# honglianghe/CDNet

Hardware: AMD Instinct MI355X
Metric: tiles/sec (train fwd+bwd+Adam), 256x256 (higher is better)
Workload: dtype fp32

## Files before the change

cdnet_amd/csrc/bn_bwd.hip:

```cpp
#include "train_util.h"
#include "bn_sums.h"

using namespace cdnet;

namespace {

struct GradIn {
    const unsigned short *g;
    int Hg, Wg;
    int oy, ox;
    int pooled;
    int coff, cstride;
};

struct BnBwdArgs {
    const unsigned short *raw;
    const unsigned short *res;
    int f16;
    const float *scale, *shift;
    int relu;
    const float *mean, *invstd;
    GradIn gin[3];
    int ngin;
    int N, H, W, C;
    float *partial;
    const float *k1, *k2, *k3;
    unsigned short *draw;
    unsigned short *dz_out;
    int rev;
};


__device__ __forceinline__ void act8_f32(const BnBwdArgs &A, size_t e, const float *sc, const float *sh, float *a, float *rawf) {
    float x[8], r[8];
    ldf8(A.raw, e, x);
    if (A.res) ldf8(A.res, e, r);
#pragma unroll
    for (int j = 0; j < 8; ++j) {
        if (rawf) rawf[j] = x[j];
        float v = A.scale ? fmaf(x[j], sc[j], sh[j]) : x[j];
        if (A.relu == 2) v = r[j];
        else {
            if (A.res) v += r[j];
            if (A.relu) v = fmaxf(v, 0.f);
// ... 286 lines not shown
                if (APPLY) {
                    if (valid) {
                        const unsigned pw = rev ? npix - 1 - p : p;
                        *reinterpret_cast<uint4 *>(A.draw + (size_t)pw * A.C + c0) = o.u;
                        if (RES) *reinterpret_cast<uint4 *>(A.dz_out + (size_t)pw * A.C + c0) = z.u;
                    }
                } else {
                    if (RES && A.dz_out && valid) *reinterpret_cast<uint4 *>(A.dz_out + (size_t)p * A.C + c0) = res[u].u;
                }
            }
        }
    });
    if (!APPLY) bn_write_partial<8>(A.partial, A.C, VPP, s1, s2);
}

template <int NG, bool RES, bool APPLY>
__global__ __launch_bounds__(256) void bn_bwd_flat32_kernel(BnBwdArgs A) {
    const int VPP = A.C / 4;
    const int slot = (int)threadIdx.x % VPP, c0 = slot * 4;
    float sc[4], sh[4], mu[4], is[4], k1[4], k2[4], k3[4], s1[4], s2[4];
    bn_load_row<4>(A.scale, c0, sc, 1.f); bn_load_row<4>(A.shift, c0, sh, 0.f); bn_load_row<4>(A.mean, c0, mu, 0.f); bn_load_row<4>(A.invstd, c0, is, 1.f);
    if (APPLY) { bn_load_row<4>(A.k1, c0, k1, 1.f); bn_load_row<4>(A.k2, c0, k2, 0.f); bn_load_row<4>(A.k3, c0, k3, 0.f); }
#pragma unroll
    for (int j = 0; j < 4; ++j) { s1[j] = 0.f; s2[j] = 0.f; }
    const unsigned npix = (unsigned)(A.N * A.H * A.W);
    const unsigned ppb = 256 / VPP, step = gridDim.x * ppb;
    const bool relu = A.relu != 0, outmask = A.relu == 2;
    const float *raw = reinterpret_cast<const float *>(A.raw), *resp = reinterpret_cast<const float *>(A.res);
    float *draw = reinterpret_cast<float *>(A.draw), *dzo = reinterpret_cast<float *>(A.dz_out);
    for (unsigned p0 = first_pixel(ppb, VPP); p0 < npix; p0 += step * BN_U) {
        f32x4 x[BN_U], r[BN_U], g[BN_U][NG];
#pragma unroll
        for (int u = 0; u < BN_U; ++u) {
            unsigned p = p0 + u * step;
            p = p < npix ? p : npix - 1;
            if (APPLY && A.rev) p = npix - 1 - p;
            x[u] = *reinterpret_cast<const f32x4 *>(raw + (size_t)p * A.C + c0);
            if (RES) r[u] = *reinterpret_cast<const f32x4 *>(resp + (size_t)p * A.C + c0);
#pragma unroll
            for (int k = 0; k < NG; ++k)
                g[u][k] = *reinterpret_cast<const f32x4 *>(reinterpret_cast<const float *>(A.gin[k].g) + (size_t)p * A.gin[k].cstride + A.gin[k].coff + c0);
        }
#pragma unroll
        for (int u = 0; u < BN_U; ++u) {
            const unsigned p = p0 + u * step;
            const bool valid = p < npix;
            f32x4 o, z;
#pragma unroll
            for (int j = 0; j < 4; ++j) {
                float v = fmaf(x[u][j], sc[j], sh[j]);
                if (RES) v = outmask ? r[u][j] : v + r[u][j];
                float gs = g[u][0][j];
#pragma unroll
                for (int k = 1; k < NG; ++k) gs += g[u][k][j];
                const float dz = (!valid || (relu && !(v > 0.f))) ? 0.f : gs;
                const float xh = (x[u][j] - mu[j]) * is[j];
                if (APPLY) { o[j] = k1[j] * (dz - k2[j] - xh * k3[j]); z[j] = dz; }
                else { s1[j] += dz; s2[j] = fmaf(dz, xh, s2[j]); z[j] = dz; }
            }
            if (APPLY && valid) {
                const unsigned pw = A.rev ? npix - 1 - p : p;
                *reinterpret_cast<f32x4 *>(draw + (size_t)pw * A.C + c0) = o;
                if (RES) *reinterpret_cast<f32x4 *>(dzo + (size_t)pw * A.C + c0) = z;
            }
            if (!APPLY && RES && dzo && valid) *reinterpret_cast<f32x4 *>(dzo + (size_t)p * A.C + c0) = z;
        }
    }
    if (!APPLY) bn_write_partial<4>(A.partial, A.C, VPP, s1, s2);
}

// ... 155 lines not shown
static int fill_bn_args(const cdnet_bn_bwd_args *a, BnBwdArgs &A, const char *who) {
    CDNET_REQUIRE(a && a->raw, "%s: null pointer", who);
    CDNET_REQUIRE(a->C % 8 == 0 && a->C >= 8 && a->C <= 2048 , "%s: C=%d unsupported", who, a->C);
    CDNET_REQUIRE(a->ngin >= 1 && a->ngin <= 3, "%s: ngin=%d", who, a->ngin);
    A.raw = a->raw; A.res = a->res; A.f16 = a->f16; A.scale = a->scale; A.shift = a->shift; A.relu = a->relu;
    A.mean = a->mean; A.invstd = a->invstd;
    for (int k = 0; k < 3; ++k) {
        A.gin[k].g = a->gin[k].g; A.gin[k].Hg = a->gin[k].Hg; A.gin[k].Wg = a->gin[k].Wg;
        A.gin[k].oy = a->gin[k].oy; A.gin[k].ox = a->gin[k].ox; A.gin[k].pooled = a->gin[k].pooled;
        A.gin[k].coff = a->gin[k].coff; A.gin[k].cstride = a->gin[k].cstride ? a->gin[k].cstride : a->C;
        if (k < a->ngin) CDNET_REQUIRE(a->gin[k].g, "%s: null gradient input %d", who, k);
        if (k < a->ngin) CDNET_REQUIRE(a->gin[k].Hg >= 1 && a->gin[k].Wg >= 1, "%s: empty gradient input %d (%d x %d)", who, k, a->gin[k].Hg, a->gin[k].Wg);
    }
    A.ngin = a->ngin; A.N = a->N; A.H = a->H; A.W = a->W; A.C = a->C;
    A.partial = nullptr; A.k1 = A.k2 = A.k3 = nullptr; A.draw = nullptr; A.dz_out = nullptr;
    return CDNET_OK;
}

enum BnPath { BN_WINDOW, BN_FLAT, BN_GENERIC };
struct BnPlan {
    BnPath path;
    bool f32;
    int nb;
    int kp, nflat;
    bool flat_sources;
};

static size_t bn_npix(const BnBwdArgs &A) { return (size_t)A.N * A.H * A.W; }

static BnPlan bn_plan_plain(const BnBwdArgs &A) {
// ... 18 lines not shown
    if (window && (!f32 || (fits32 && A.shift && A.invstd))) P.path = BN_WINDOW;
    else if (flat && (!f32 || fits32)) P.path = BN_FLAT;
    const int V = f32 && P.path != BN_GENERIC ? 4 : 8;
    P.nb = window ? bn_grid((size_t)A.N * ((A.H + 1) / 2) * ((A.W + 1) / 2), A.C, V, 1) : bn_grid(bn_npix(A), A.C, V, BN_U);
    return P;
}

static thread_local int g_bn_last_plan[2] = {0, 0};
static thread_local int g_bn_last_pass = 0;

static int bn_plan_record(const BnPlan &P, const BnBwdArgs &A, bool apply, bool dz_source) {
    const int path = P.path == BN_WINDOW ? CDNET_BN_PATH_WINDOW : P.path == BN_FLAT ? CDNET_BN_PATH_FLAT : CDNET_BN_PATH_GENERIC;
    const int n = P.path == BN_WINDOW ? P.nflat : P.path == BN_FLAT ? A.ngin : 0;
    const int res = P.path == BN_FLAT && A.res ? 1 : 0;
    const int kp = P.path == BN_WINDOW ? P.kp : 0;
    return path | (P.f32 ? 1 : 0) << 2 | n << 3 | res << 5 | kp << 6 | (apply ? 1 : 0) << 8 | (dz_source ? 1 : 0) << 9 | P.nb << 10;
}

template <bool APPLY>
static void launch(const BnPlan &P, const BnBwdArgs &A, hipStream_t st, bool dz_source = false) {
    g_bn_last_plan[APPLY ? 1 : 0] = bn_plan_record(P, A, APPLY, dz_source);
    g_bn_last_pass = APPLY ? 1 : 0;
    auto window = [&](auto nf) {
        constexpr int NF = decltype(nf)::value;
        if (P.f32) bn_bwd_window32_kernel<NF, APPLY><<<P.nb, 256, 0, st>>>(A, P.kp);
        else bn_bwd_window_kernel<NF, APPLY><<<P.nb, 256, 0, st>>>(A, P.kp);
    };
    auto flat = [&](auto ng, auto res) {
        constexpr int NG = decltype(ng)::value;
        constexpr bool RES = decltype(res)::value;
        if (P.f32) bn_bwd_flat32_kernel<NG, RES, APPLY><<<P.nb, 256, 0, st>>>(A);
        else bn_bwd_flat_kernel<NG, RES, APPLY><<<P.nb, 256, 0, st>>>(A);
    };
    using std::integral_constant;
    using std::true_type;
    using std::false_type;
    switch (P.path) {
        case BN_WINDOW:
            if (P.nflat == 0) window(integral_constant<int, 0>{});
            else if (P.nflat == 1) window(integral_constant<int, 1>{});
            else window(integral_constant<int, 2>{});
            break;
        case BN_FLAT:
            switch (A.ngin * 2 + (A.res ? 1 : 0)) {
                case 2: flat(integral_constant<int, 1>{}, false_type{}); break;
                case 3: flat(integral_constant<int, 1>{}, true_type{}); break;
// ... 24 lines not shown
    B.gin[0].coff = 0; B.gin[0].cstride = A.C;
    B.res = nullptr; B.relu = 0; B.dz_out = nullptr;
    return B;
}

extern "C" int cdnet_bn_backward(const cdnet_bn_bwd_args *a, const float *gamma, float *dgamma, float *dbeta, float *workspace,
                                 size_t workspace_floats, uint16_t *draw, uint16_t *dz_out, void *stream) {
    BnBwdArgs A;
    int rc = fill_bn_args(a, A, "cdnet_bn_backward");
    if (rc) return rc;
    hipStream_t st = (hipStream_t)stream;
    const size_t npix = bn_npix(A);
    CDNET_REQUIRE(npix * (size_t)A.C < ((size_t)1 << 32) && npix < ((size_t)1 << 31), "cdnet_bn_backward: tensor too large for 32-bit pixel indexing");
    const BnPlan P = bn_plan(A, draw, dz_out);
    CDNET_REQUIRE(A.relu != 2 || (P.flat_sources && A.res), "cdnet_bn_backward: relu = 2 (mask from the stored output) needs same-size gradient sources and res");
    static const bool dz_reuse = !(getenv("CDNET_BN_DZ_REUSE") && atoi(getenv("CDNET_BN_DZ_REUSE")) == 0);
    const bool reuse = dz_reuse && P.path == BN_FLAT && A.mean && A.res && dz_out;
    A.draw = draw;
    A.rev = 1;
    if (A.mean) {
        CDNET_REQUIRE(gamma && A.invstd && workspace, "cdnet_bn_backward: BatchNorm layer needs gamma/invstd/workspace");
        const size_t need = (size_t)P.nb * 2 * A.C + 3 * (size_t)A.C;
        if (workspace_floats < need) { set_error("cdnet_bn_backward: workspace %zu < %zu floats", workspace_floats, need); return CDNET_E_WORKSPACE; }
        A.partial = workspace;
        A.dz_out = dz_reuse ? dz_out : nullptr;
        float *k = workspace + (size_t)P.nb * 2 * A.C;
        launch<false>(P, A, st);
        bn_finalize(A, A.partial, P.nb, gamma, dgamma, dbeta, k, st);
        bn_set_coeffs(A, k);
    }
// ... 59 lines not shown
```

cdnet_amd/csrc/conv.hip:

```cpp
#include <type_traits>
#include <vector>
#include "common.h"
#include "conv_args.h"
#include "launch.h"
#include "xform.h"
#include "stage16.h"
#include <stdlib.h>

using namespace cdnet;

namespace {

__device__ int g_dbg_dummy;

struct PackDesc {
    const float *w;
    unsigned short *out;
    int Cout, Cin, KH, KW, CK, BN, nchunk, ntile, TAPS, mode, parity;
    unsigned block0, nblocks;
    int split;
    const float *scale;
};

__device__ __forceinline__ void pack_range(const PackDesc &d, size_t first, size_t stride) {
// ... 1324 lines not shown
    CDNET_REQUIRE(A.N > 0 && A.H > 0 && A.W > 0 && A.Cout > 0 && A.Cout % 8 == 0, "cdnet_conv_forward: bad size (Cout must be a multiple of 8)");
    {
        int ctot_xf = 0;
        for (int i = 0; i < A.nsrc; ++i) ctot_xf += A.src[i].C;
        CDNET_REQUIRE(ctot_xf <= XF_MAX, "cdnet_conv_forward: %d source channels exceed the %d-entry scale/shift table", ctot_xf, XF_MAX);
    }
    CDNET_REQUIRE(A.ws == 0 || A.ws == 2, "cdnet_conv_forward: ws must be 0 or 2 (BatchNorm-backward statistics epilogue)");
    if (A.f32) {
        CDNET_REQUIRE(A.f32 == 1, "cdnet_conv_forward: f32 must be 0 or 1");
        for (int i = 0; i < A.nsrc; ++i)
            CDNET_REQUIRE(A.src[i].f16 == 2, "cdnet_conv_forward(f32): every source must be fp32 (f16 = 2)");
    } else {
        for (int i = 0; i < A.nsrc; ++i)
            CDNET_REQUIRE(A.src[i].f16 == 0 || A.src[i].f16 == 1, "cdnet_conv_forward: fp32 sources need args.f32 = 1");
    }
    if (A.eres && A.ws != 2) {
        CDNET_REQUIRE(A.ostride == 1 && A.npar == 1 && A.out_coff == 0 && A.out_cstride == A.Cout && !A.stats && !A.orelu &&
                      !A.out_f16 && ((A.eres_scale == nullptr) == (A.eres_shift == nullptr)),
                      "cdnet_conv_forward: fused residual epilogue needs a dense bf16 output, no statistics and no ReLU before the add");
    }
    int nchunk = 0;
    for (int i = 0; i < A.nsrc; ++i) {
        CDNET_REQUIRE(A.src[i].x && A.src[i].C % A.CK == 0, "cdnet_conv_forward: source %d channels %d not a multiple of CK=%d",
                      i, A.src[i].C, A.CK);
        CDNET_REQUIRE(!(A.src[i].pool && A.src[i].res), "cdnet_conv_forward: pool+residual source unsupported");
        nchunk += A.src[i].C / A.CK;
    }
    const bool padded = A.nchunk == nchunk + 1 && A.taps == 9 && A.nsrc == 2 && !A.f32;
    CDNET_REQUIRE(nchunk == A.nchunk || padded, "cdnet_conv_forward: nchunk %d != %d", A.nchunk, nchunk);
    CDNET_REQUIRE((A.taps == 9 && A.npar == 1 && A.ostride == 1) || (A.taps == 1 && A.npar == 1 && A.ostride == 1) ||
// ... 56 lines not shown
```

cdnet_amd/csrc/conv32.hip:

```cpp
#include <type_traits>
#include "common.h"
#include "conv_args.h"
#include "launch.h"
#include "split_bf16.h"
#include <stdlib.h>

using namespace cdnet;

namespace {

constexpr int CK = 16;
constexpr int PSTR = CK * 2 + 16;
constexpr int XF_MAX = 2048;

template <int TH, int TW, int BN, int TAPS>
struct Lds32 {
    static constexpr int NPIX = (TH + 2) * (TW + 2);
    static constexpr int A_PLANE = NPIX * PSTR;
    static constexpr int B_PLANE = TAPS * CK * BN * 2;
    static constexpr int STAGE = 2 * A_PLANE + 2 * B_PLANE;
    static constexpr int STATS_BYTES = 4 * 2 * BN * 4;
    static constexpr int MAIN = ((STAGE > STATS_BYTES ? STAGE : STATS_BYTES) + 15) / 16 * 16;
    static int bytes(int ctot) { return MAIN + 2 * ((ctot + 7) / 8 * 8) * 4; }
};
// ... 348 lines not shown
    const int smem = L::bytes(ctot);
    dim3 grid(cdiv(A.W, TW) * cdiv(A.H, TH) * A.N * A.npar, cdiv(A.Cout, BN), 1);
    g_conv_last_form = conv_form(CDNET_CONV_FAMILY_F32, BN, TAPS, 0, false, false, false, 0, 0, TH);
    return launch_lds<conv_f32_kernel<TH, TW, BN, WM, WN, TAPS>>(grid, 256, L::bytes(XF_MAX), smem, st, "hipFuncSetAttribute(conv32)", "conv_f32_kernel", A);
}

template <int TAPS>
int dispatch_conv32(const ConvArgs &A, hipStream_t st) {
    if (A.tile == 16 && A.BN == 64) return launch_conv32<16, 16, 64, 4, 1, TAPS>(A, st);
    if (A.tile == 16 && A.BN == 32) return launch_conv32<16, 16, 32, 4, 1, TAPS>(A, st);
    if (A.tile == 8 && A.BN == 64) return launch_conv32<8, 8, 64, 2, 2, TAPS>(A, st);
    set_error("cdnet_conv_forward(f32): unsupported configuration tile=%d CK=%d BN=%d", A.tile, A.CK, A.BN);
    return CDNET_E_ARG;
}

template <int BN, int NCH, bool XF, bool ERES>
__global__ __launch_bounds__(256, 4) void conv1x1_f32_stream_kernel(ConvArgs A) {
    constexpr int NPW = BN / 32;
    constexpr int B_PLANE = CK * BN * 2;
    constexpr int CIN = NCH * CK;
    __shared__ __attribute__((aligned(16))) unsigned char smem[NCH * 2 * B_PLANE + 2 * CIN * 4];
    unsigned char *lds_b = smem;
    float *s_xf = reinterpret_cast<float *>(smem + NCH * 2 * B_PLANE);

    const int tid = threadIdx.x, lane = tid & 63, wave = __builtin_amdgcn_readfirstlane(tid >> 6);
    const int half = lane >> 5, l31 = lane & 31;
    const int cout_tile = blockIdx.y, cout0 = cout_tile * BN;
    const ConvSrc &S = A.src[0];
    {
        const u32x4 *wsrc = reinterpret_cast<const u32x4 *>(A.w + (size_t)cout_tile * NCH * B_PLANE);
        u32x4 *bdst = reinterpret_cast<u32x4 *>(lds_b);
        for (int v = tid; v < NCH * 2 * B_PLANE / 16; v += 256) bdst[v] = wsrc[v];
// ... 83 lines not shown
        const size_t left = P - (size_t)blk * 32, rows = left < 32 ? left : 32;
        const __amdgpu_buffer_rsrc_t ro = rsrc(obase + (size_t)blk * 32 * cs4, rows * cs4);
        float ev[NPW][16];
        if (ERES) {
            const __amdgpu_buffer_rsrc_t re = rsrc(ebase + (size_t)blk * 32 * ce4, rows * ce4);
#pragma unroll
            for (int ni = 0; ni < NPW; ++ni)
#pragma unroll
                for (int r = 0; r < 16; ++r) {
                    const unsigned pr = (r & 3) + 8 * (r >> 2);
                    ev[ni][r] = __builtin_bit_cast(float, TAIL ? __builtin_amdgcn_raw_buffer_load_b32(re, (int)(vo_eres[ni] + pr * ce4), 0, 0)
                                                               : __builtin_amdgcn_raw_buffer_load_b32(re, (int)vo_eres[ni], (int)(pr * ce4), 0));
                }
        }
#pragma unroll
        for (int ni = 0; ni < NPW; ++ni)
#pragma unroll
            for (int r = 0; r < 16; ++r) {
                const unsigned pr = (r & 3) + 8 * (r >> 2);
                float v = fmaf(acc[ni][r], osc[ni], osh[ni]);
                v = orelu ? fmaxf(v, 0.f) : v;
                if (ERES) {
                    v = fmaf(ev[ni][r], esc[ni], esh[ni]) + v;
                    v = eres_relu ? fmaxf(v, 0.f) : v;
                }
                if (TAIL) __builtin_amdgcn_raw_buffer_store_b32(__builtin_bit_cast(unsigned, v), ro, (int)(vo_out[ni] + pr * cs4), 0, 0);
                else __builtin_amdgcn_raw_buffer_store_b32(__builtin_bit_cast(unsigned, v), ro, (int)vo_out[ni], (int)(pr * cs4), 0);
            }
    };
    f32x4 xa[NCH][2], xb[NCH][2];
    const int nfull = (int)(P / 32);
    if (blk < nfull) {
        request(xa, blk);
#pragma unroll
        for (int c = 0; c < NCH; ++c) asm volatile("" ::"v"(xa[c][0]), "v"(xa[c][1]));
        for (;;) {
            block(std::false_type{}, xa, xb);
            blk += bstride;
            if (blk >= nfull) break;
            block(std::false_type{}, xb, xa);
            blk += bstride;
            if (blk >= nfull) break;
        }
// ... 3 lines not shown
        block(std::true_type{}, xa, xb);
    }
}

template <int BN, int NCH>
int launch_conv1x1_stream(const ConvArgs &A, hipStream_t st) {
    int n_cu = 0;
    if (const int rc = cu_count(&n_cu)) return rc;
    const long long nblk = ((long long)A.N * A.H * A.W + 31) / 32;
    const int ctiles = cdiv(A.Cout, BN);
    const long long waves = (long long)n_cu * 16 / ctiles > 4 ? (long long)n_cu * 16 / ctiles : 4;
    const long long rounds = (nblk + waves - 1) / waves;
    const long long G = ((nblk + rounds - 1) / rounds + 3) / 4;
    dim3 grid((unsigned)G, ctiles, 1);
    return with_bool(A.src[0].scale != nullptr, [&](auto xf_c) {
        return with_bool(A.eres != nullptr, [&](auto er_c) {
            g_conv_last_form = conv_form(CDNET_CONV_FAMILY_STREAM, BN, 1, decltype(xf_c)::value ? 1 : 0, false, false, false, 0, 0, 16, 16, NCH, decltype(er_c)::value);
            conv1x1_f32_stream_kernel<BN, NCH, decltype(xf_c)::value, decltype(er_c)::value><<<grid, 256, 0, st>>>(A);
            return check_launch("conv1x1_f32_stream_kernel");
        });
    });
}

int try_conv1x1_stream(const ConvArgs &A, hipStream_t st) {
    if (A.debug & CONV_DBG_NO_STREAM_1X1) return -1;
    if (A.taps != 1 || A.taps1 != 0 || A.npar != 1 || A.ostride != 1 || A.ws || A.stats || A.pool_out || A.nsrc != 1) return -1;
    const ConvSrc &s = A.src[0];
    if (s.off_y || s.off_x || s.Hs != A.H || s.Ws != A.W || (s.row_stride && s.row_stride != s.Ws * s.C) || s.pool || s.res) return -1;
    if (s.relu && !s.scale) return -1;
    if (s.C != A.nchunk * CK || (long long)A.N * A.H * A.W > (1LL << 31) - 64 || (long long)A.out_cstride * 4 * 36 >= (1LL << 31)) return -1;
    auto go = [&](auto bn_c) -> int {
        constexpr int BN = decltype(bn_c)::value;
        if (A.nchunk == 1) return launch_conv1x1_stream<BN, 1>(A, st);
        if (A.nchunk == 2) return launch_conv1x1_stream<BN, 2>(A, st);
        if (A.nchunk == 4) return launch_conv1x1_stream<BN, 4>(A, st);
        return -1;
    };
    if (A.BN == 64) return go(std::integral_constant<int, 64>{});
    if (A.BN == 32) return go(std::integral_constant<int, 32>{});
    return -1;
}

__global__ __launch_bounds__(256) void materialize_f32_kernel(const ConvSrc s, int N, int H, int W, float *__restrict__ out) {
    const int VPP = s.C / 4;
    const size_t total = (size_t)N * H * W * VPP;
// ... 42 lines not shown
            }
        }
        *reinterpret_cast<float4 *>(out + pix * s.C + c) = val;
    }
}

}

namespace cdnet {

int conv_forward_f32(const ConvArgs &A, hipStream_t st) {
    CDNET_REQUIRE(A.CK == 16, "cdnet_conv_forward(f32): CK must be 16 (got %d)", A.CK);
    for (int i = 0; i < A.nsrc; ++i)
        CDNET_REQUIRE(!A.src[i].pool, "cdnet_conv_forward(f32): pooled sources must be materialised (cdnet_src_materialize)");
    CDNET_REQUIRE(!A.out_f16, "cdnet_conv_forward(f32): out_f16 must be 0");
    {
        const int rc = conv_forward_f32_ws(A, st);
        if (rc >= 0) return rc;
    }
    CDNET_REQUIRE(A.ws != 2, "cdnet_conv_forward(f32): the BatchNorm-backward statistics epilogue (ws = 2) needs the producer / consumer kernel "
                             "(ask cdnet_conv_ws_eligible first)");
    CDNET_REQUIRE(A.taps1 == 0 || A.taps1 == A.taps, "cdnet_conv_forward(f32): a one-tap second source runs on conv_ws32_kernel only (ask cdnet_conv_ws_eligible)");
    CDNET_REQUIRE(!A.pool_out, "cdnet_conv_forward(f32): the fused max-pool output rides in conv_ws32_kernel's epilogue only (ask cdnet_conv_ws_eligible)");
    if (A.taps == 9) return dispatch_conv32<9>(A, st);
    if (A.taps == 4) return dispatch_conv32<4>(A, st);
    {
        const int rc = try_conv1x1_stream(A, st);
        if (rc >= 0) return rc;
    }
    return dispatch_conv32<1>(A, st);
// ... 12 lines not shown
```

cdnet_amd/csrc/conv_args.h:

```cpp
#pragma once
#include "../../include/cdnet_hip.h"

struct ConvSrc {
    const unsigned short *x;
    const unsigned short *res;
    const float *scale;
    const float *shift;
    int C, Hs, Ws, pool, relu, off_y, off_x;
    int f16, row_stride;
};

struct ConvArgs {
    ConvSrc src[2];
    int nsrc;
    const unsigned short *w;
    const float *bias;
    const float *oscale;
    const float *oshift;
    int orelu;
    unsigned short *out;
    int Cout, out_cstride, out_coff;
    float *stats;
    int N, H, W;
    int taps, npar, ostride, nchunk;
    int tile, CK, BN;
    int out_f16;
    int debug;
    int ws;
    int f32;
    const unsigned short *eres;
    const float *eres_scale, *eres_shift;
    int eres_f16, eres_relu;
    int taps1, pad_;
    unsigned short *pool_out;
    const float *dot_w, *dot_b;
    float *dot_out;
};

enum : int {
    CONV_DBG_WS16_QUAD = 16,
    CONV_DBG_ONE_TILE = 32,
    CONV_DBG_PERSIST_SMALL = 64,
    CONV_DBG_OLD_WS16 = 128,
    CONV_DBG_NO_STREAM_1X1 = 256,
    CONV_DBG_GRID_SHIFT = 8,
};
enum : int {
    WGRAD_DBG_NO_WS = 8,
    WGRAD_DBG_ALL_QUADS = 16,
};

// ... 17 lines not shown
```

cdnet_amd/engine.py:

```python
import ctypes as C
import os
import torch

from . import _lib


class ConvSrc(C.Structure):
    _fields_ = [('x', C.c_void_p), ('res', C.c_void_p), ('scale', C.c_void_p), ('shift', C.c_void_p),
                ('C', C.c_int), ('Hs', C.c_int), ('Ws', C.c_int), ('pool', C.c_int), ('relu', C.c_int),
                ('off_y', C.c_int), ('off_x', C.c_int), ('f16', C.c_int), ('row_stride', C.c_int)]


class ConvArgs(C.Structure):
    _fields_ = [('src', ConvSrc * 2), ('nsrc', C.c_int), ('w', C.c_void_p), ('bias', C.c_void_p),
                ('oscale', C.c_void_p), ('oshift', C.c_void_p), ('orelu', C.c_int), ('out', C.c_void_p),
                ('Cout', C.c_int), ('out_cstride', C.c_int), ('out_coff', C.c_int), ('stats', C.c_void_p),
                ('N', C.c_int), ('H', C.c_int), ('W', C.c_int), ('taps', C.c_int), ('npar', C.c_int),
                ('ostride', C.c_int), ('nchunk', C.c_int), ('tile', C.c_int), ('CK', C.c_int), ('BN', C.c_int),
                ('out_f16', C.c_int), ('debug', C.c_int), ('ws', C.c_int), ('f32', C.c_int),
                ('eres', C.c_void_p), ('eres_scale', C.c_void_p), ('eres_shift', C.c_void_p), ('eres_f16', C.c_int), ('eres_relu', C.c_int),
                ('taps1', C.c_int), ('pad_', C.c_int), ('pool_out', C.c_void_p),
                ('dot_w', C.c_void_p), ('dot_b', C.c_void_p), ('dot_out', C.c_void_p)]


def _dp(t):
    return None if t is None else t.data_ptr()


class Src:

    def __init__(self, x, scale=None, shift=None, relu=False, pool=False, res=None, off=(0, 0), view=None):
        assert x.dtype in (torch.bfloat16, torch.float16, torch.float32) and x.is_contiguous()
        assert res is None or res.dtype == x.dtype
        self.x, self.scale, self.shift, self.relu, self.pool, self.res, self.off = x, scale, shift, relu, pool, res, off
        if view is None:
            assert x.dim() == 4
            self.N, self.Hs, self.Ws, self.Cc = x.shape
# ... 140 lines not shown
    if cout_scale is not None:
        assert mode == 0 and cout_scale.dtype == torch.float32 and cout_scale.numel() == Cout
        _lib.call('cdnet_pack_conv_weights_scaled', _lib.ptr(w), _lib.ptr(cout_scale), _lib.ptr(out), Cout, Cin, KH, KW, CK, BN,
                  mode | (PACK_SPLIT if split else 0), _lib.stream_ptr())
        return out
    _lib.call('cdnet_pack_conv_weights', _lib.ptr(w), _lib.ptr(out), Cout, Cin, KH, KW, CK, BN, mode | (PACK_SPLIT if split else 0),
              _lib.stream_ptr())
    return out


CONV_DEBUG = 0


def conv_forward(srcs, wpacked, Cout, cfg, taps=9, transposed=False, bias=None, oscale=None, oshift=None,
                 orelu=False, out=None, stats=None, H=None, W=None, out_dtype=torch.bfloat16, eres=None, query_ws=False, bns=None, taps1=0, pool_out=None, dot=None,
                 pad_chunks=0, debug_or=0, out_coff=0):
    tile, CK, BN = cfg[:3]
    s0 = srcs[0]
    f32 = s0.f32
    assert all(s.f32 == f32 for s in srcs)
    if f32:
        out_dtype = torch.float32
    N = s0.N
    if H is None:
        H, W = s0.logical_hw()
        H, W = H + 0, W + 0
    ostride = 2 if transposed else 1
    npar = 4 if transposed else 1
    a = ConvArgs()
    nchunk = 0
    for i, s in enumerate(srcs):
# ... 25 lines not shown
    a.debug = CONV_DEBUG | debug_or
    a.f32 = int(f32)
    assert out is None or (out.dtype == torch.float32) == f32
    if eres is not None:
        assert not transposed and stats is None and not orelu and out.dtype == (torch.float32 if f32 else torch.bfloat16) and tuple(eres.x.shape) == tuple(out.shape)
        assert eres.f32 == f32
        a.eres, a.eres_scale, a.eres_shift = eres.x.data_ptr(), _dp(eres.scale), _dp(eres.shift)
        a.eres_f16, a.eres_relu = int(eres.f16), int(eres.relu)
    if bns is not None:
        raw, sc, sh, mu, inv, partial = bns
        assert eres is None and stats is None and bias is None and oscale is None and oshift is None and tuple(raw.shape) == tuple(out.shape)
        a.ws = 2
        a.eres, a.oscale, a.oshift, a.eres_scale, a.eres_shift, a.stats = raw.data_ptr(), sc.data_ptr(), sh.data_ptr(), mu.data_ptr(), inv.data_ptr(), partial.data_ptr()
    if query_ws:
        return int(_lib.load().cdnet_conv_ws_eligible(C.byref(a)))
    _lib.call('cdnet_conv_forward', C.byref(a), _lib.stream_ptr())
    return out, stats
```

cdnet_amd/runtime.py:

```python
import ctypes as C
import weakref
import torch

from . import _lib, engine
from .engine import Src

BN_EPS = 1e-5
BN_MOMENTUM = 0.1

import os as _os

PRECISION = _os.environ.get('CDNET_PRECISION', 'bf16')
assert PRECISION in ('bf16', 'fp32'), PRECISION


def set_precision(p):
    global PRECISION
    assert p in ('bf16', 'fp32'), p
    if p != PRECISION:
        PRECISION = p
        WEIGHTS_EPOCH[0] += 1


def act_dtype():
# ... 198 lines not shown
                return Src(out), Src(pout)
        return self.forward(srcs, False), None

    def forward(self, srcs, training, relu=True, H=None, W=None, out_dtype=None, eres=None, debug_or=0):
        if PRECISION == 'fp32':
            out_dtype = torch.float32
        elif out_dtype is None:
            out_dtype = torch.bfloat16
        if H is None:
            H, W = srcs[0].logical_hw()
        if DEBUG_NORELU:
            relu = False
        self.prepare([s.C for s in srcs], H, W, srcs[0].N)
        bias = None if self.bias is None else self.bias.detach()
        if self.bn is None:
            out, _ = engine.conv_forward(srcs, self.wp, self.Cout, self.cfg, self.taps, self.transposed, bias=bias, H=H, W=W,
                                         out_dtype=out_dtype, eres=eres)
            if training:
                self.saved = (srcs, out, H, W)
                self.node_relu, self.node_res = False, None
                if TAPE is not None:
                    TAPE.append(self)
            return Src(out)
        if not training:
            ep = self.eval_pack([s.C for s in srcs])
            if ep is not None:
                out, _ = engine.conv_forward(srcs, ep[0], self.Cout, self.cfg, self.taps, self.transposed, oshift=ep[1],
                                             orelu=relu and eres is None, H=H, W=W, out_dtype=out_dtype, eres=eres, debug_or=debug_or)
                return Src(out)
            sc, sh = self.eval_fold()
            out, _ = engine.conv_forward(srcs, self.wp, self.Cout, self.cfg, self.taps, self.transposed, oscale=sc,
                                         oshift=sh, orelu=relu and eres is None, H=H, W=W, out_dtype=out_dtype, eres=eres, debug_or=debug_or)
# ... 128 lines not shown


def input_pack(x):
    assert x.dtype == torch.float32 and x.is_cuda and x.dim() == 4
    x = x.contiguous()
    N, Cc, H, W = x.shape
    out = torch.empty((N, H, W, 16), dtype=act_dtype(), device=x.device)
    _lib.call(_lib.entry('cdnet_input_pack', PRECISION == 'fp32'), _lib.ptr(x), N, Cc, H, W, _lib.ptr(out),
              _lib.stream_ptr())
    return out


POOL_MATERIALIZE = True
RU_MATERIALIZE = True
RU_FUSE = True
EVAL_FOLD_WEIGHTS = True
RU_EVAL_ONE_LAUNCH = True
RU_EVAL_POINT_DOT = True


class PointLogit:

    def __init__(self, point):
        self.point = point


def residual_unit_eval(c1, c2, cr, x, relu2=True, dot=None):
    if not (RU_EVAL_ONE_LAUNCH and EVAL_FOLD_WEIGHTS) or not getattr(c2, 'fold_eval', True) or x.pool or x.C % 16 or c2.Cout % 16:
        return None
    H, W = x.logical_hw()
# ... 74 lines not shown
```

cdnet_amd/trainer.py:

```python
import ctypes as C
import os

import torch

from . import _lib, engine, optim, runtime, streams
from .allreduce import BucketReducer, bucketed_allreduce
from .engine import Src
from .optim import HEAD_PARAMS, FlatState
from .synth import synthetic_batch


class GradIn(C.Structure):
    _fields_ = [('g', C.c_void_p), ('Hg', C.c_int), ('Wg', C.c_int), ('oy', C.c_int), ('ox', C.c_int),
                ('pooled', C.c_int), ('coff', C.c_int), ('cstride', C.c_int), ('pad_', C.c_int)]


class BnBwdArgs(C.Structure):
    _fields_ = [('raw', C.c_void_p), ('res', C.c_void_p), ('scale', C.c_void_p), ('shift', C.c_void_p),
                ('mean', C.c_void_p), ('invstd', C.c_void_p), ('gin', GradIn * 3), ('ngin', C.c_int),
                ('f16', C.c_int), ('relu', C.c_int), ('N', C.c_int), ('H', C.c_int), ('W', C.c_int), ('C', C.c_int)]


_WGRAD_WGS_DEEP, _WGRAD_WGS_SHALLOW = 128, 160
_WGRAD_WGS_KQ = 128
_WGRAD_WGS_F32 = 160
_RU_1X1_SIDE = True
WGRAD_STREAM = True
HEAD_BWD_FUSE = True
_WGRAD_DEFER = 0x100
_WGRAD_DEEP_HW = 16384


class _on_stream:
    __slots__ = ('s', 'prev')

    def __init__(self, s):
        self.s = s

    def __enter__(self):
        self.prev = torch.cuda.current_stream()
        torch.cuda.set_stream(self.s)

# ... 62 lines not shown
        self._wss = {}
        self.losses = torch.zeros((11,), dtype=torch.float32, device=self.dev)
        self.alpha = 0.0
        self.dice, self.weight_map = 1, 1
        self.loss_var = torch.full((1,), -1.0, dtype=torch.float32, device=self.dev)
        self.boundary = 0
        self.loss_boundary = torch.zeros((1,), dtype=torch.float32, device=self.dev)
        self.tape = []
        self._cat_cache = {}
        self._wstream, self._events = None, {}
        self.ar_stats = None
        self._packb_pending = False
        self._packb_stream = True
        self._side_active = False
        self.head_fused = False
        self._rd_mb = float(os.environ.get('CDNET_WGRAD_REDUCE_MB', '300'))
        self._rd_pending, self._rd_params, self._rd_bytes, self._rd_tables = [], [], 0, {}
        self._forwards, self._bn_base = 0, 0
        if world_size > 1:
            self.sync_from_rank0()

    def sync_from_rank0(self, src=0):
        import torch.distributed as dist
        if not (dist.is_available() and dist.is_initialized()) or dist.get_world_size() == 1:
            return
        f = self.flat
        works = [dist.broadcast(t, src=src, async_op=True) for t in (f.P, f.M, f.V, f.S) if t is not None]
        meta = torch.tensor([float(f.step_count), float(self._bn_base + self._forwards)], dtype=torch.float64, device=self.dev)
        works.append(dist.broadcast(meta, src=src, async_op=True))
        bufs = [b for b in self.model.buffers() if b.is_floating_point()]
# ... 60 lines not shown
                d = None
            elif len(gl) == 1 and not gl[0].coff and gl[0].cstride in (0, o.shape[3]):
                d = gl[0].t
            else:
                d = self.buf(('dcat', key), o.shape, runtime.act_dtype())
                self.grad_sum(gl, None, o.shape[0] * o.shape[1] * o.shape[2], o.shape[3], d)
            self._cat_cache[key] = d
        return self._cat_cache[key]

    def forward(self, x):
        m = self.model
        m.train()
        self._forwards += 1
        runtime.TAPE = self.tape
        del self.tape[:]
        try:
            out = m(x)
        finally:
            runtime.TAPE = None
        return out

    def loss_and_grads(self, mask, point, direction, label, dirlab, point_t, weight):
        B, _, H, W = mask.shape
        lib = _lib.load()
        ND = direction.shape[1]
        ws = self._ws('loss', lib.cdnet_dam_loss_classes_workspace_floats(B, H * W, ND))
        dmask = self.buf('dmask', mask.shape, torch.float32)
        dpoint = self.buf('dpoint', point.shape, torch.float32)
        ddir = self.buf('ddir', direction.shape, torch.float32)
        assert label.dtype == torch.uint8 and dirlab.dtype == torch.uint8 and weight.dtype == torch.uint8
        assert point_t.dtype == torch.float16
        if self.dice != 1:
            raise ValueError('dice = %r with a DAM model: the reference dies on an unbound loss_direction_dice (train_util_dam.py:297); only 1 works'
                             % (self.dice,))
        from .utils import loss_terms
# ... 98 lines not shown
        def add(t, g):
            grads.setdefault(id(t), []).append(g)
        for t, g in heads:
            add(t, g)
        self._overlap_begin()
        self._overlap_done(params)
        self._backward_tape(grads, add)

    def _backward_tape(self, grads, add):
        self._cat_cache = {}
        self._rd_pending, self._rd_params, self._rd_bytes = [], [], 0
        if len(self._rd_tables) > 16:
            self._rd_tables.clear()
        self._readers, self._producer, self._bn_partials = {}, {}, {}
        self._tape_pos = {id(Lt): k for k, Lt in enumerate(self.tape)}
        for Lt in self.tape:
            if isinstance(Lt, runtime.FuseNode):
                for t in Lt.saved[0]:
                    self._readers[id(t.x)] = self._readers.get(id(t.x), 0) + 1
                continue
            for sx in Lt.saved[0]:
                self._readers[id(sx.x)] = self._readers.get(id(sx.x), 0) + 1
                if sx.res is not None:
                    self._readers[id(sx.res)] = self._readers.get(id(sx.res), 0) + 1
            self._producer[id(Lt.saved[1])] = Lt
        side = self._side_stream()
        self._side_active = side is not None
        if self._packb_pending:
            torch.cuda.current_stream().wait_event(self._event('packb'))
            self._packb_pending = False
# ... 2 lines not shown
                L.backward(self, grads, add)
                continue
            gl = self.take(grads, id(L.saved[1]))
            if gl is None:
                continue
            owner = getattr(L, 'fused_res_of', None)
            if owner is not None:
                grads.setdefault(id(owner.saved[1]), []).extend(gl)
                owner.deferred_layer = L
                continue
            self._layer_backward(k, L, gl, grads, add, side)
            d = getattr(L, 'deferred_layer', None)
            if d is not None:
                L.deferred_layer = None
                self._layer_backward(('deferred', k), d, self.take(grads, id(d.saved[1])), grads, add, side)
        if side is not None:
            with _on_stream(side):
                self._flush_reduces()
            ev = self._event(-1)
            ev.record(side)
            torch.cuda.current_stream().wait_event(ev)
        else:
            self._flush_reduces()

    def _weights_done(self, params):
        if not self._rd_pending:
            self._overlap_done(params)
            return
        self._rd_params.append(params)
        if self._rd_bytes >= self._rd_mb * (1 << 20):
# ... 121 lines not shown
        a.relu = relu
        a.N, a.H, a.W, a.C = out.shape
        return a

    def _bn_backward(self, L, out, gl, add):
        No, Ho, Wo, Co = out.shape
        res = getattr(L, 'node_res', None)
        has_bn = L.bn is not None
        if len(gl) > 3:
            plain = [g for g in gl if not g.pooled and g.oy == 0 and g.ox == 0 and (g.Hg, g.Wg) == (Ho, Wo)]
            rest = [g for g in gl if g not in plain]
            assert len(rest) <= 2 and len(plain) >= 2, (L.name, len(gl))
            d = self.buf(('gsum', L.name), (No, Ho, Wo, Co), runtime.act_dtype())
            self.grad_sum(plain, None, No * Ho * Wo, Co, d)
            gl = rest + [_G(d, Ho, Wo)]
        a = self._bn_args(L, out, gl, res, int(getattr(L, 'node_relu', True)))
        draw = self.buf(('draw', L.name), (No, Ho, Wo, Co), runtime.act_dtype())
        dz = None
        if res is not None:
            dz = self.buf(('dz', L.name), (No, Ho, Wo, Co), runtime.act_dtype())
        ws = self._ws('bn', _lib.load().cdnet_bn_backward_workspace_floats(Co))
        bn = L.bn
        _lib.call('cdnet_bn_backward', C.byref(a), _lib.ptr(bn.weight.detach()) if has_bn else None,
                  _lib.ptr(bn.weight.grad) if has_bn else None, _lib.ptr(bn.bias.grad) if has_bn else None,
                  _lib.ptr(ws), ws.numel(), _lib.ptr(draw), _lib.ptr(dz), _lib.stream_ptr())
        if res is not None:
            add(getattr(L, 'node_res_grad_to', None) if getattr(L, 'node_res_grad_to', None) is not None else res, _G(dz, Ho, Wo))
            L.node_res_grad_to = None
        return draw

    def _side_stream(self):
# ... 344 lines not shown
```

include/cdnet_hip.h:

```cpp
#ifndef CDNET_HIP_H
#define CDNET_HIP_H

#include <stddef.h>
#include <stdint.h>

#ifdef __cplusplus
extern "C" {
#endif

#define CDNET_OK            0
#define CDNET_E_ARG         1
#define CDNET_E_WORKSPACE   2
#define CDNET_E_LAUNCH      3

#define CDNET_ABI_VERSION   5

int         cdnet_abi_version(void);
size_t      cdnet_abi_sizeof(const char *struct_name);
const char *cdnet_last_error(void);
const char *cdnet_build_info(void);
int         cdnet_spin(int microseconds, void *stream);
int         cdnet_box_copy(const void *src, void *dst, size_t bytes, void *stream);
int         cdnet_box_mfma(const uint32_t *seed, float *sink, unsigned long long *stamps, int workgroups, int waves_per_wg, int iters, void *stream);

// ... 78 lines not shown
    int nchunk;
    int tile, CK, BN;
    int out_f16;
    int debug;
    int ws;
    int f32;
    const uint16_t *eres;
    const float *eres_scale, *eres_shift;
    int eres_f16, eres_relu;
    int taps1;
    int pad_;
    uint16_t *pool_out;
    const float *dot_w;
    const float *dot_b;
    float *dot_out;
} cdnet_conv_args;

size_t cdnet_conv_packed_weight_elems(int Cout, int nchunk, int taps, int CK, int BN, int npar);
#define CDNET_PACK_SPLIT 16
int cdnet_pack_conv_weights(const float *w, void *packed, int Cout, int Cin, int KH, int KW, int CK, int BN, int mode,
                            void *stream);
int cdnet_pack_conv_weights_scaled(const float *w, const float *cout_scale, void *packed, int Cout, int Cin, int KH, int KW, int CK,
                                   int BN, int mode, void *stream);
typedef struct cdnet_pack_job {
    const float *w;
    void *packed;
    int Cout, Cin, KH, KW, CK, BN, mode, pad_;
} cdnet_pack_job;
size_t cdnet_pack_batch_table_bytes(int n_jobs);
int cdnet_pack_conv_weights_batch(const cdnet_pack_job *jobs, int n_jobs, void *table, size_t table_bytes, int upload,
                                  void *stream);
int cdnet_conv_forward(const cdnet_conv_args *args, void *stream);

#define CDNET_CONV_FAMILY_FWD    1
#define CDNET_CONV_FAMILY_WS     2
#define CDNET_CONV_FAMILY_WS16   3
#define CDNET_CONV_FAMILY_F32    4
#define CDNET_CONV_FAMILY_STREAM 5
#define CDNET_CONV_FAMILY_WS32   6
int cdnet_conv_forward_last_form(void);

typedef struct cdnet_dilated_conv_args {
    const void *in;
    const void *w;
    const float *scale;
    const float *shift;
    void *out;
    int N, H, W;
// ... 148 lines not shown
    int oy, ox;
    int pooled;
    int coff, cstride;
    int pad_;
} cdnet_grad_in;

typedef struct cdnet_bn_bwd_args {
    const uint16_t *raw;
    const uint16_t *res;
    const float *scale, *shift;
    const float *mean, *invstd;
    cdnet_grad_in gin[3];
    int ngin;
    int f16, relu;
    int N, H, W, C;
} cdnet_bn_bwd_args;

size_t cdnet_bn_backward_workspace_floats(int C);
int cdnet_bn_backward_stats(const cdnet_bn_bwd_args *args, const float *gamma, float *dgamma, float *dbeta, float *workspace,
                            size_t workspace_floats, float *ktab, void *stream);
int cdnet_bn_backward_apply(const cdnet_bn_bwd_args *args, const float *ktab, uint16_t *draw, void *stream);
int cdnet_bn_backward_finalize(const cdnet_bn_bwd_args *args, const float *gamma, float *dgamma, float *dbeta, const float *partial,
                               int nb, float *ktab, void *stream);
int cdnet_bn_backward(const cdnet_bn_bwd_args *args, const float *gamma, float *dgamma, float *dbeta, float *workspace,
                      size_t workspace_floats, uint16_t *draw, uint16_t *dz_out, void *stream);

#define CDNET_BN_PATH_WINDOW  1
#define CDNET_BN_PATH_FLAT    2
#define CDNET_BN_PATH_GENERIC 3
int cdnet_bn_backward_last_plan(void);
// ... 165 lines not shown
```

Measured before the change: 1092.

## Store residual ReLU mask as a bit plane in fp32 conv and read it in BN backward

The fused 1x1 stream conv's residual+ReLU epilogue now also writes a 1-bit-per-channel ReLU mask, packed with ballots and lane writes. The fp32 flat BN backward kernel reads these bits instead of the full fp32 stored output, cutting its residual read traffic from 32 bits to 1 bit per element. The trainer wires the plane through forward and backward and stops allocating it for layers where backward never used it. The cost is an extra small store and some lane shuffling in the conv epilogue, plus more plumbing and eligibility checks.

Result: no change. 1099, median of 6 (+0.6%).

```diff
diff --git a/cdnet_amd/csrc/bn_bwd.hip b/cdnet_amd/csrc/bn_bwd.hip
--- a/cdnet_amd/csrc/bn_bwd.hip
+++ b/cdnet_amd/csrc/bn_bwd.hip
@@ -28,6 +28,7 @@
     unsigned short *draw;
     unsigned short *dz_out;
     int rev;
+    const unsigned char *mask_bits;
 };
 
 
@@ -344,8 +345,9 @@
     if (!APPLY) bn_write_partial<8>(A.partial, A.C, VPP, s1, s2);
 }
 
-template <int NG, bool RES, bool APPLY>
+template <int NG, bool RES, bool APPLY, bool BITS = false>
 __global__ __launch_bounds__(256) void bn_bwd_flat32_kernel(BnBwdArgs A) {
+    static_assert(!BITS || RES, "the mask plane stands in for the stored output of the residual form");
     const int VPP = A.C / 4;
     const int slot = (int)threadIdx.x % VPP, c0 = slot * 4;
     float sc[4], sh[4], mu[4], is[4], k1[4], k2[4], k3[4], s1[4], s2[4];
@@ -358,15 +360,19 @@
     const bool relu = A.relu != 0, outmask = A.relu == 2;
     const float *raw = reinterpret_cast<const float *>(A.raw), *resp = reinterpret_cast<const float *>(A.res);
     float *draw = reinterpret_cast<float *>(A.draw), *dzo = reinterpret_cast<float *>(A.dz_out);
+    const unsigned char *mbits = A.mask_bits + (c0 >> 3);
+    const unsigned mrow = (unsigned)A.C >> 3, msh = c0 & 4;
     for (unsigned p0 = first_pixel(ppb, VPP); p0 < npix; p0 += step * BN_U) {
         f32x4 x[BN_U], r[BN_U], g[BN_U][NG];
+        unsigned mb[BN_U];
 #pragma unroll
         for (int u = 0; u < BN_U; ++u) {
             unsigned p = p0 + u * step;
             p = p < npix ? p : npix - 1;
             if (APPLY && A.rev) p = npix - 1 - p;
             x[u] = *reinterpret_cast<const f32x4 *>(raw + (size_t)p * A.C + c0);
-            if (RES) r[u] = *reinterpret_cast<const f32x4 *>(resp + (size_t)p * A.C + c0);
+            if (RES && !BITS) r[u] = *reinterpret_cast<const f32x4 *>(resp + (size_t)p * A.C + c0);
+            if (BITS) mb[u] = mbits[(size_t)p * mrow];
 #pragma unroll
             for (int k = 0; k < NG; ++k)
                 g[u][k] = *reinterpret_cast<const f32x4 *>(reinterpret_cast<const float *>(A.gin[k].g) + (size_t)p * A.gin[k].cstride + A.gin[k].coff + c0);
@@ -379,11 +385,12 @@
 #pragma unroll
             for (int j = 0; j < 4; ++j) {
                 float v = fmaf(x[u][j], sc[j], sh[j]);
-                if (RES) v = outmask ? r[u][j] : v + r[u][j];
+                if (RES && !BITS) v = outmask ? r[u][j] : v + r[u][j];
                 float gs = g[u][0][j];
 #pragma unroll
                 for (int k = 1; k < NG; ++k) gs += g[u][k][j];
-                const float dz = (!valid || (relu && !(v > 0.f))) ? 0.f : gs;
+                const float dz = BITS ? ((valid && ((mb[u] >> (msh + j)) & 1u)) ? gs : 0.f)
+                                      : ((!valid || (relu && !(v > 0.f))) ? 0.f : gs);
                 const float xh = (x[u][j] - mu[j]) * is[j];
                 if (APPLY) { o[j] = k1[j] * (dz - k2[j] - xh * k3[j]); z[j] = dz; }
                 else { s1[j] += dz; s2[j] = fmaf(dz, xh, s2[j]); z[j] = dz; }
@@ -569,6 +576,8 @@
     }
     A.ngin = a->ngin; A.N = a->N; A.H = a->H; A.W = a->W; A.C = a->C;
     A.partial = nullptr; A.k1 = A.k2 = A.k3 = nullptr; A.draw = nullptr; A.dz_out = nullptr;
+    A.mask_bits = a->relu == 3 ? a->mask_bits : nullptr;
+    CDNET_REQUIRE(a->relu != 3 || a->mask_bits, "%s: relu = 3 needs mask_bits", who);
     return CDNET_OK;
 }
 
@@ -617,7 +626,8 @@
     const int n = P.path == BN_WINDOW ? P.nflat : P.path == BN_FLAT ? A.ngin : 0;
     const int res = P.path == BN_FLAT && A.res ? 1 : 0;
     const int kp = P.path == BN_WINDOW ? P.kp : 0;
-    return path | (P.f32 ? 1 : 0) << 2 | n << 3 | res << 5 | kp << 6 | (apply ? 1 : 0) << 8 | (dz_source ? 1 : 0) << 9 | P.nb << 10;
+    return path | (P.f32 ? 1 : 0) << 2 | n << 3 | res << 5 | kp << 6 | (apply ? 1 : 0) << 8 | (dz_source ? 1 : 0) << 9 | P.nb << 10 |
+           (A.relu == 3 ? 1 : 0) << 22;
 }
 
 template <bool APPLY>
@@ -632,7 +642,8 @@
     auto flat = [&](auto ng, auto res) {
         constexpr int NG = decltype(ng)::value;
         constexpr bool RES = decltype(res)::value;
-        if (P.f32) bn_bwd_flat32_kernel<NG, RES, APPLY><<<P.nb, 256, 0, st>>>(A);
+        if (P.f32 && RES && A.relu == 3) bn_bwd_flat32_kernel<NG, true, APPLY, true><<<P.nb, 256, 0, st>>>(A);
+        else if (P.f32) bn_bwd_flat32_kernel<NG, RES, APPLY><<<P.nb, 256, 0, st>>>(A);
         else bn_bwd_flat_kernel<NG, RES, APPLY><<<P.nb, 256, 0, st>>>(A);
     };
     using std::integral_constant;
@@ -687,6 +698,8 @@
     CDNET_REQUIRE(npix * (size_t)A.C < ((size_t)1 << 32) && npix < ((size_t)1 << 31), "cdnet_bn_backward: tensor too large for 32-bit pixel indexing");
     const BnPlan P = bn_plan(A, draw, dz_out);
     CDNET_REQUIRE(A.relu != 2 || (P.flat_sources && A.res), "cdnet_bn_backward: relu = 2 (mask from the stored output) needs same-size gradient sources and res");
+    CDNET_REQUIRE(A.relu != 3 || (P.flat_sources && A.res && P.path == BN_FLAT && P.f32),
+                  "cdnet_bn_backward: relu = 3 (mask from the bit plane) needs what relu = 2 needs and the fp32 flat kernels (f16 = 2, C <= 1024, draw and dz_out)");
     static const bool dz_reuse = !(getenv("CDNET_BN_DZ_REUSE") && atoi(getenv("CDNET_BN_DZ_REUSE")) == 0);
     const bool reuse = dz_reuse && P.path == BN_FLAT && A.mean && A.res && dz_out;
     A.draw = draw;
diff --git a/cdnet_amd/csrc/conv.hip b/cdnet_amd/csrc/conv.hip
--- a/cdnet_amd/csrc/conv.hip
+++ b/cdnet_amd/csrc/conv.hip
@@ -1362,6 +1362,7 @@
         for (int i = 0; i < A.nsrc; ++i)
             CDNET_REQUIRE(A.src[i].f16 == 0 || A.src[i].f16 == 1, "cdnet_conv_forward: fp32 sources need args.f32 = 1");
     }
+    CDNET_REQUIRE(!A.eres_mask || A.f32, "cdnet_conv_forward: eres_mask (the ReLU mask as a bit plane) exists in fp32 mode only");
     if (A.eres && A.ws != 2) {
         CDNET_REQUIRE(A.ostride == 1 && A.npar == 1 && A.out_coff == 0 && A.out_cstride == A.Cout && !A.stats && !A.orelu &&
                       !A.out_f16 && ((A.eres_scale == nullptr) == (A.eres_shift == nullptr)),
diff --git a/cdnet_amd/csrc/conv32.hip b/cdnet_amd/csrc/conv32.hip
--- a/cdnet_amd/csrc/conv32.hip
+++ b/cdnet_amd/csrc/conv32.hip
@@ -386,8 +386,15 @@
     return CDNET_E_ARG;
 }
 
-template <int BN, int NCH, bool XF, bool ERES>
+template <int LANE>
+__device__ __forceinline__ int write_lane(int old, unsigned v) {
+    asm("v_writelane_b32 %0, %1, %2" : "+v"(old) : "s"(v), "n"(LANE));
+    return old;
+}
+
+template <int BN, int NCH, bool XF, bool ERES, bool MASK = false>
 __global__ __launch_bounds__(256, 4) void conv1x1_f32_stream_kernel(ConvArgs A) {
+    static_assert(!MASK || ERES, "the mask plane belongs to the fused residual epilogue");
     constexpr int NPW = BN / 32;
     constexpr int B_PLANE = CK * BN * 2;
     constexpr int CIN = NCH * CK;
@@ -501,7 +508,8 @@
                 }
         }
 #pragma unroll
-        for (int ni = 0; ni < NPW; ++ni)
+        for (int ni = 0; ni < NPW; ++ni) {
+            unsigned long long bal[16];
 #pragma unroll
             for (int r = 0; r < 16; ++r) {
                 const unsigned pr = (r & 3) + 8 * (r >> 2);
@@ -513,7 +521,22 @@
                 }
                 if (TAIL) __builtin_amdgcn_raw_buffer_store_b32(__builtin_bit_cast(unsigned, v), ro, (int)(vo_out[ni] + pr * cs4), 0, 0);
                 else __builtin_amdgcn_raw_buffer_store_b32(__builtin_bit_cast(unsigned, v), ro, (int)vo_out[ni], (int)(pr * cs4), 0);
-            }
+                if (MASK) bal[r] = __ballot(v > 0.f);
+            }
+            if (MASK) {
+                int mword = 0;
+                [&]<int... R>(std::integer_sequence<int, R...>) {
+                    ((mword = write_lane<R>(mword, (unsigned)bal[R]), mword = write_lane<32 + R>(mword, (unsigned)(bal[R] >> 32))), ...);
+                }(std::make_integer_sequence<int, 16>{});
+                const unsigned mrow = (unsigned)cout >> 3;
+                const __amdgpu_buffer_rsrc_t rm = rsrc(reinterpret_cast<const char *>(A.eres_mask) + (size_t)blk * 32 * mrow, rows * mrow);
+                unsigned ml = (unsigned)lane;
+                asm volatile("" : "+v"(ml));
+                const unsigned mp = (ml & 3) + 8 * ((ml >> 2) & 3) + 4 * (ml >> 5);
+                const unsigned mo = ((ml & 31) < 16 && cout0 + ni * 32 < cout) ? mp * mrow + ((unsigned)(cout0 + ni * 32) >> 3) : 0x7fff0000u;
+                __builtin_amdgcn_raw_buffer_store_b32((unsigned)mword, rm, (int)mo, 0, 0);
+            }
+        }
     };
     f32x4 xa[NCH][2], xb[NCH][2];
     const int nfull = (int)(P / 32);
@@ -547,9 +570,15 @@
     const long long G = ((nblk + rounds - 1) / rounds + 3) / 4;
     dim3 grid((unsigned)G, ctiles, 1);
     return with_bool(A.src[0].scale != nullptr, [&](auto xf_c) {
+        constexpr bool XF = decltype(xf_c)::value;
+        if (A.eres_mask) {
+            g_conv_last_form = conv_form(CDNET_CONV_FAMILY_STREAM, BN, 1, XF ? 1 : 0, false, false, false, 0, 0, 16, 16, NCH, true) | CDNET_CONV_FORM_ERES_MASK;
+            conv1x1_f32_stream_kernel<BN, NCH, XF, true, true><<<grid, 256, 0, st>>>(A);
+            return check_launch("conv1x1_f32_stream_kernel");
+        }
         return with_bool(A.eres != nullptr, [&](auto er_c) {
-            g_conv_last_form = conv_form(CDNET_CONV_FAMILY_STREAM, BN, 1, decltype(xf_c)::value ? 1 : 0, false, false, false, 0, 0, 16, 16, NCH, decltype(er_c)::value);
-            conv1x1_f32_stream_kernel<BN, NCH, decltype(xf_c)::value, decltype(er_c)::value><<<grid, 256, 0, st>>>(A);
+            g_conv_last_form = conv_form(CDNET_CONV_FAMILY_STREAM, BN, 1, XF ? 1 : 0, false, false, false, 0, 0, 16, 16, NCH, decltype(er_c)::value);
+            conv1x1_f32_stream_kernel<BN, NCH, XF, decltype(er_c)::value><<<grid, 256, 0, st>>>(A);
             return check_launch("conv1x1_f32_stream_kernel");
         });
     });
@@ -562,6 +591,7 @@
     if (s.off_y || s.off_x || s.Hs != A.H || s.Ws != A.W || (s.row_stride && s.row_stride != s.Ws * s.C) || s.pool || s.res) return -1;
     if (s.relu && !s.scale) return -1;
     if (s.C != A.nchunk * CK || (long long)A.N * A.H * A.W > (1LL << 31) - 64 || (long long)A.out_cstride * 4 * 36 >= (1LL << 31)) return -1;
+    if (A.eres_mask && (!A.eres || !A.eres_relu || A.Cout % 32 != 0 || A.out_coff != 0 || A.out_cstride != A.Cout)) return -1;
     auto go = [&](auto bn_c) -> int {
         constexpr int BN = decltype(bn_c)::value;
         if (A.nchunk == 1) return launch_conv1x1_stream<BN, 1>(A, st);
@@ -634,6 +664,12 @@
     for (int i = 0; i < A.nsrc; ++i)
         CDNET_REQUIRE(!A.src[i].pool, "cdnet_conv_forward(f32): pooled sources must be materialised (cdnet_src_materialize)");
     CDNET_REQUIRE(!A.out_f16, "cdnet_conv_forward(f32): out_f16 must be 0");
+    if (A.eres_mask) {
+        const int rc = try_conv1x1_stream(A, st);
+        if (rc >= 0) return rc;
+        set_error("cdnet_conv_forward(f32): eres_mask needs conv1x1_f32_stream_kernel (one dense 1x1 source of 1 / 2 / 4 chunks, eres with its ReLU, Cout %% 32 == 0): call again without it");
+        return CDNET_E_ARG;
+    }
     {
         const int rc = conv_forward_f32_ws(A, st);
         if (rc >= 0) return rc;
diff --git a/cdnet_amd/csrc/conv_args.h b/cdnet_amd/csrc/conv_args.h
--- a/cdnet_amd/csrc/conv_args.h
+++ b/cdnet_amd/csrc/conv_args.h
@@ -35,6 +35,7 @@
     unsigned short *pool_out;
     const float *dot_w, *dot_b;
     float *dot_out;
+    unsigned char *eres_mask;
 };
 
 enum : int {
diff --git a/cdnet_amd/engine.py b/cdnet_amd/engine.py
--- a/cdnet_amd/engine.py
+++ b/cdnet_amd/engine.py
@@ -20,7 +20,7 @@
                 ('out_f16', C.c_int), ('debug', C.c_int), ('ws', C.c_int), ('f32', C.c_int),
                 ('eres', C.c_void_p), ('eres_scale', C.c_void_p), ('eres_shift', C.c_void_p), ('eres_f16', C.c_int), ('eres_relu', C.c_int),
                 ('taps1', C.c_int), ('pad_', C.c_int), ('pool_out', C.c_void_p),
-                ('dot_w', C.c_void_p), ('dot_b', C.c_void_p), ('dot_out', C.c_void_p)]
+                ('dot_w', C.c_void_p), ('dot_b', C.c_void_p), ('dot_out', C.c_void_p), ('eres_mask', C.c_void_p)]
 
 
 def _dp(t):
@@ -191,7 +191,7 @@
 
 def conv_forward(srcs, wpacked, Cout, cfg, taps=9, transposed=False, bias=None, oscale=None, oshift=None,
                  orelu=False, out=None, stats=None, H=None, W=None, out_dtype=torch.bfloat16, eres=None, query_ws=False, bns=None, taps1=0, pool_out=None, dot=None,
-                 pad_chunks=0, debug_or=0, out_coff=0):
+                 pad_chunks=0, debug_or=0, out_coff=0, eres_mask=None):
     tile, CK, BN = cfg[:3]
     s0 = srcs[0]
     f32 = s0.f32
@@ -247,5 +247,16 @@
         a.eres, a.oscale, a.oshift, a.eres_scale, a.eres_shift, a.stats = raw.data_ptr(), sc.data_ptr(), sh.data_ptr(), mu.data_ptr(), inv.data_ptr(), partial.data_ptr()
     if query_ws:
         return int(_lib.load().cdnet_conv_ws_eligible(C.byref(a)))
+    if eres_mask is not None:
+        assert eres is not None and f32 and eres_mask.dtype == torch.uint8 and eres_mask.numel() == N * H * W * (Cout // 8)
+        a.eres_mask = eres_mask.data_ptr()
+        rc = _lib.load().cdnet_conv_forward(C.byref(a), _lib.stream_ptr())
+        if rc != 1:
+            _lib.check(rc, 'cdnet_conv_forward')
+            return out, stats
+        a.eres_mask = None
     _lib.call('cdnet_conv_forward', C.byref(a), _lib.stream_ptr())
     return out, stats
+
+
+CONV_FORM_ERES_MASK = 1 << 27
diff --git a/cdnet_amd/runtime.py b/cdnet_amd/runtime.py
--- a/cdnet_amd/runtime.py
+++ b/cdnet_amd/runtime.py
@@ -236,8 +236,13 @@
         self.prepare([s.C for s in srcs], H, W, srcs[0].N)
         bias = None if self.bias is None else self.bias.detach()
         if self.bn is None:
+            plane = None
+            if training and eres is not None and eres.relu and MASK_PLANE is not None and PRECISION == 'fp32' and self.Cout % 32 == 0:
+                plane = MASK_PLANE(self, (srcs[0].N * H * W, self.Cout // 8))
             out, _ = engine.conv_forward(srcs, self.wp, self.Cout, self.cfg, self.taps, self.transposed, bias=bias, H=H, W=W,
-                                         out_dtype=out_dtype, eres=eres)
+                                         out_dtype=out_dtype, eres=eres, eres_mask=plane)
+            wrote = plane is not None and bool(_lib.load().cdnet_conv_forward_last_form() & engine.CONV_FORM_ERES_MASK)
+            self.eres_mask = plane if wrote else None
             if training:
                 self.saved = (srcs, out, H, W)
                 self.node_relu, self.node_res = False, None
@@ -396,6 +401,7 @@
 POOL_MATERIALIZE = True
 RU_MATERIALIZE = True
 RU_FUSE = True
+MASK_PLANE = None
 EVAL_FOLD_WEIGHTS = True
 RU_EVAL_ONE_LAUNCH = True
 RU_EVAL_POINT_DOT = True
diff --git a/cdnet_amd/trainer.py b/cdnet_amd/trainer.py
--- a/cdnet_amd/trainer.py
+++ b/cdnet_amd/trainer.py
@@ -18,7 +18,7 @@
 class BnBwdArgs(C.Structure):
     _fields_ = [('raw', C.c_void_p), ('res', C.c_void_p), ('scale', C.c_void_p), ('shift', C.c_void_p),
                 ('mean', C.c_void_p), ('invstd', C.c_void_p), ('gin', GradIn * 3), ('ngin', C.c_int),
-                ('f16', C.c_int), ('relu', C.c_int), ('N', C.c_int), ('H', C.c_int), ('W', C.c_int), ('C', C.c_int)]
+                ('f16', C.c_int), ('relu', C.c_int), ('N', C.c_int), ('H', C.c_int), ('W', C.c_int), ('C', C.c_int), ('mask_bits', C.c_void_p)]
 
 
 _WGRAD_WGS_DEEP, _WGRAD_WGS_SHALLOW = 128, 160
@@ -26,6 +26,7 @@
 _WGRAD_WGS_F32 = 160
 _RU_1X1_SIDE = True
 WGRAD_STREAM = True
+RU_MASK_BITS = os.environ.get('CDNET_RU_MASK_BITS', '1') != '0'
 HEAD_BWD_FUSE = True
 _WGRAD_DEFER = 0x100
 _WGRAD_DEEP_HW = 16384
@@ -118,6 +119,8 @@
         self._packb_stream = True
         self._side_active = False
         self.head_fused = False
+        self.mask_bits_used = []
+        self._mask_skip = set()
         self._rd_mb = float(os.environ.get('CDNET_WGRAD_REDUCE_MB', '300'))
         self._rd_pending, self._rd_params, self._rd_bytes, self._rd_tables = [], [], 0, {}
         self._forwards, self._bn_base = 0, 0
@@ -208,11 +211,19 @@
         self._forwards += 1
         runtime.TAPE = self.tape
         del self.tape[:]
+        if RU_MASK_BITS and runtime.PRECISION == 'fp32':
+            runtime.MASK_PLANE = self._mask_plane
         try:
             out = m(x)
         finally:
             runtime.TAPE = None
+            runtime.MASK_PLANE = None
         return out
+
+    def _mask_plane(self, L, shape):
+        if L.name in self._mask_skip:
+            return None
+        return self.buf(('maskbits', L.name), shape, torch.uint8)
 
     def loss_and_grads(self, mask, point, direction, label, dirlab, point_t, weight):
         B, _, H, W = mask.shape
@@ -341,6 +352,7 @@
             self._rd_tables.clear()
         self._readers, self._producer, self._bn_partials = {}, {}, {}
         self._tape_pos = {id(Lt): k for k, Lt in enumerate(self.tape)}
+        self.mask_bits_used = []
         for Lt in self.tape:
             if isinstance(Lt, runtime.FuseNode):
                 for t in Lt.saved[0]:
@@ -373,6 +385,9 @@
             if d is not None:
                 L.deferred_layer = None
                 self._layer_backward(('deferred', k), d, self.take(grads, id(d.saved[1])), grads, add, side)
+        for Lt in self.tape:
+            if getattr(Lt, 'eres_mask', None) is not None and Lt.name not in self.mask_bits_used:
+                self._mask_skip.add(Lt.name)
         if side is not None:
             with _on_stream(side):
                 self._flush_reduces()
@@ -524,7 +539,16 @@
             d = self.buf(('gsum', L.name), (No, Ho, Wo, Co), runtime.act_dtype())
             self.grad_sum(plain, None, No * Ho * Wo, Co, d)
             gl = rest + [_G(d, Ho, Wo)]
-        a = self._bn_args(L, out, gl, res, int(getattr(L, 'node_relu', True)))
+        relu = int(getattr(L, 'node_relu', True))
+        d = getattr(L, 'deferred_layer', None)
+        bits = getattr(d, 'eres_mask', None) if d is not None and relu == 2 and d.saved[1] is res else None
+        if bits is not None and (out.dtype != torch.float32 or Co > 1024 or bits.numel() != No * Ho * Wo * (Co // 8)
+                                 or any(g.pooled or g.oy or g.ox or (g.Hg, g.Wg) != (Ho, Wo) for g in gl)):
+            bits = None
+        a = self._bn_args(L, out, gl, res, 3 if bits is not None else relu)
+        if bits is not None:
+            a.mask_bits = bits.data_ptr()
+            self.mask_bits_used.append(d.name)
         draw = self.buf(('draw', L.name), (No, Ho, Wo, Co), runtime.act_dtype())
         dz = None
         if res is not None:
diff --git a/include/cdnet_hip.h b/include/cdnet_hip.h
--- a/include/cdnet_hip.h
+++ b/include/cdnet_hip.h
@@ -116,6 +116,7 @@
     const float *dot_w;
     const float *dot_b;
     float *dot_out;
+    uint8_t *eres_mask;
 } cdnet_conv_args;
 
 size_t cdnet_conv_packed_weight_elems(int Cout, int nchunk, int taps, int CK, int BN, int npar);
@@ -134,6 +135,7 @@
                                   void *stream);
 int cdnet_conv_forward(const cdnet_conv_args *args, void *stream);
 
+#define CDNET_CONV_FORM_ERES_MASK (1 << 27)
 #define CDNET_CONV_FAMILY_FWD    1
 #define CDNET_CONV_FAMILY_WS     2
 #define CDNET_CONV_FAMILY_WS16   3
@@ -312,6 +314,7 @@
     int ngin;
     int f16, relu;
     int N, H, W, C;
+    const uint8_t *mask_bits;
 } cdnet_bn_bwd_args;
 
 size_t cdnet_bn_backward_workspace_floats(int C);
```
